# NjuHaoZhang/AMMCNet_AAAI2021

Hardware: AMD Instinct MI355X
Metric: frames/sec, 256x256x4 dual-stream clips (twostream forward, inference) (higher is better)
Workload: dtype f32-equivalent: (hi,lo) f16 split, 3 fp16 MFMAs per product (v_mfma_f32_32x32x16_f16 in the 4-wave k-half-major kernels, 16x16x32 in the 8-wave / fused-decoder kernels), f32 accumulate; 1 GPU; Ped2 full dual-stream + 2000-slot memory module, batch=16, inference (BASELINE.json configs[1]); batch_per_gpu=16, frame=256x256, n_embed=2000, embed_dim=64, k=2, parallelism=replicas x1 (no collective)

## Files before the change

ammcnet_aaai2021_amd/csrc/conv_outc_s16.hip:

```cpp
#include "ammc_common.h"
#include <hip/hip_fp16.h>
#include <stdio.h>
#include <stdlib.h>

namespace ammc_s16 {

typedef _Float16 f16x8o __attribute__((ext_vector_type(8)));

constexpr float O_LO_INV = 1.f / 2048.f;
constexpr int O_TH = 8, O_TW = 32, O_HW = O_TW + 2, O_HP = (O_TH + 2) * O_HW;
constexpr int O_APIECES = O_HP * 8;
constexpr int O_NT = 512;
constexpr int O_R = (O_APIECES + O_NT - 1) / O_NT;
constexpr int O_ASTAGE = ((O_APIECES + 63) / 64) * 64 * 4;
constexpr int O_MAXNS = 4;
constexpr int O_TG = O_MAXNS * 256;
constexpr int O_NS = 3;
constexpr int O_MAXCC = 2;
static_assert(O_R == 6, "OUTC_WAIT below knows 0, 2, 6 and 8 outstanding operations");

struct OutcArgs {
  AmmcConvDesc d;
  int tiles_x, tiles_y, ncc, kpad, total, nstore;
};

#define OUTC_WAIT(n)                                                              \
  switch (n) {                                                                    \
    case 0: asm volatile("s_waitcnt vmcnt(0)" ::: "memory"); break;               \
    case 2: asm volatile("s_waitcnt vmcnt(2)" ::: "memory"); break;               \
    case 6: asm volatile("s_waitcnt vmcnt(6)" ::: "memory"); break;               \
    default: asm volatile("s_waitcnt vmcnt(8)" ::: "memory"); break;              \
  }

__global__ __launch_bounds__(O_NT, 1) void conv_outc_s16_kernel(OutcArgs a) {
  extern __shared__ __attribute__((aligned(16))) float smem[];
  float* As = smem;
  float* Fs = smem + O_NS * O_ASTAGE;
  float* Tg = Fs + 9 * O_MAXCC * 128;
  float* Scr = Tg + 2 * O_TG;
  float* Sq = Scr + 256;

  const int tid = threadIdx.x, lane = tid & 63, wave = tid >> 6;
  const int l15 = lane & 15, g4 = lane >> 4;
  const AmmcConvDesc& d = a.d;
  const int G = gridDim.x;
  const int first = ammc_xcd_remap(blockIdx.x, G);
  const int ntile = (a.total - first + G - 1) / G;
  const int U = ntile * a.ncc;

  for (int i = tid; i < 9 * a.ncc * 32; i += O_NT) {
    const int chunk = i >> 5, row = (i >> 3) & 3, q = i & 7;
    int sl = q ^ row;
    sl ^= (sl >> 1) & 1;
    const f32x4 w = *reinterpret_cast<const f32x4*>(d.w + (int64_t)row * a.kpad + chunk * 32 + 4 * sl);
    *reinterpret_cast<f32x4*>(Fs + chunk * 128 + row * 32 + 4 * q) = w;
  }

  const int ns = a.nstore;
  const int64_t ycs = d.y_cs > 0 ? d.y_cs : 1;
  const bool score = d.sq_target != nullptr;

  float sc = 1.f, sh = 0.f;
  if (g4 < ns) {
    if (d.scale) sc = d.scale[g4];
    if (d.shift) sh = d.shift[g4];
  }
  asm volatile("" : "+v"(sc), "+v"(sh));

  int a_off[O_R];
#pragma unroll
  for (int j = 0; j < O_R; ++j) {
    int p = j * O_NT + tid;
    p = p < O_APIECES ? p : O_APIECES - 1;
    const int hp = p >> 3;
    int ls = (p & 7) ^ (hp & 7);
    ls ^= (ls >> 1) & 1;
    const int hy = hp / O_HW;
    const int hx = hp - hy * O_HW;
    a_off[j] = (int)((int64_t)hy * d.x_rs + (int64_t)hx * d.x_ps) + 4 * ls;
  }
#define OUTC_ISSUE(tile_, cc_, stage_)                                                                            \
  {                                                                                                               \
    int sp_ = (tile_);                                                                                            \
    const int tx_ = sp_ % a.tiles_x;                                                                              \
    sp_ /= a.tiles_x;                                                                                             \
    const int ty_ = sp_ % a.tiles_y;                                                                              \
    const int b_ = sp_ / a.tiles_y;                                                                               \
    const float* xp_ = d.x + ((int64_t)b_ * d.x_bs + (int64_t)(ty_ * O_TH) * d.x_rs + (int64_t)(tx_ * O_TW) * d.x_ps) + (cc_) * 32; \
    float* dst_ = As + (stage_) * O_ASTAGE + wave * 256;                                                          \
    _Pragma("unroll") for (int j = 0; j < O_R; ++j)                                                               \
      __builtin_amdgcn_global_load_lds(xp_ + a_off[j], (j * O_NT + wave * 64) * 4 < O_ASTAGE ? dst_ + j * O_NT * 4 : Scr, 16, 0, 0); \
  }
  const int tg_e0 = tid < ns * 256 ? tid : 0, tg_e1 = 512 + tid < ns * 256 ? 512 + tid : 0;
  const int64_t tg_o0 = (tg_e0 >> 8) * ycs + ((tg_e0 >> 5) & 7) * d.y_rs + (tg_e0 & 31) * d.y_ps;
  const int64_t tg_o1 = (tg_e1 >> 8) * ycs + ((tg_e1 >> 5) & 7) * d.y_rs + (tg_e1 & 31) * d.y_ps;
#define OUTC_ISSUE_TG(tile_, buf_)                                                                                \
  {                                                                                                               \
    int sp_ = (tile_);                                                                                            \
    const int tx_ = sp_ % a.tiles_x;                                                                              \
    sp_ /= a.tiles_x;                                                                                             \
    const int ty_ = sp_ % a.tiles_y;                                                                              \
    const int b_ = sp_ / a.tiles_y;                                                                               \
    const float* tp_ = d.sq_target + ((int64_t)b_ * d.y_bs + (int64_t)(ty_ * O_TH) * d.y_rs + (int64_t)(tx_ * O_TW) * d.y_ps); \
    __builtin_amdgcn_global_load_lds(tp_ + tg_o0, wave * 64 < ns * 256 ? Tg + (buf_) * O_TG + wave * 64 : Scr, 4, 0, 0);   \
    __builtin_amdgcn_global_load_lds(tp_ + tg_o1, 512 + wave * 64 < ns * 256 ? Tg + (buf_) * O_TG + 512 + wave * 64 : Scr, 4, 0, 0); \
  }

  int i_tile = first, i_cc = 0, i_stage = 0, issued = 0;
#define OUTC_ISSUE_NEXT()                                         \
  {                                                               \
    OUTC_ISSUE(i_tile, i_cc, i_stage);                            \
    ++issued;                                                     \
    i_stage = i_stage + 1 == O_NS ? 0 : i_stage + 1;              \
    if (++i_cc == a.ncc) i_cc = 0, i_tile += G;                   \
  }
  if (score && a.ncc == 1 && U > 0) OUTC_ISSUE_TG(first, 0);
  if (issued < U) OUTC_ISSUE_NEXT();
  if (issued < U) OUTC_ISSUE_NEXT();

  const int slot_hi = 2 * g4 + (g4 & 1), slot_lo = slot_hi ^ 1;
  const int frow = l15 & 3;
  const float* f_hi = Fs + frow * 32 + ((slot_hi ^ frow) << 2);
  const float* f_lo = Fs + frow * 32 + ((slot_lo ^ frow) << 2);
  const int hpb = wave * O_HW + l15;
  f32x4 acc[2], acx[2];
  acc[0] = acc[1] = acx[0] = acx[1] = f32x4{0.f, 0.f, 0.f, 0.f};
  int c_tile = first, c_cc = 0, c_stage = 0, c_par = 0;
  bool pend = false;
  int pend_b = 0;
  asm volatile("s_waitcnt lgkmcnt(0)" ::: "memory");

  for (int u = 0; u < U; ++u) {
    const int nwait = (u + 1 < U ? O_R : 0) + (pend ? 2 : 0);
    OUTC_WAIT(nwait);
    __builtin_amdgcn_s_barrier();
    asm volatile("" ::: "memory");
    if (pend && score && tid == 0) {
      float s = 0.f;
#pragma unroll
      for (int w = 0; w < 8; ++w) s += Sq[(c_par ^ 1) * 8 + w];
      unsafeAtomicAdd(d.sq_acc + pend_b, s);
    }
    const bool last_cc = c_cc + 1 == a.ncc;
    int sp = c_tile;
    const int tx = sp % a.tiles_x;
    sp /= a.tiles_x;
    const int ty = sp % a.tiles_y;
    const int b = sp / a.tiles_y;
    if (score && u + 1 < U && (a.ncc == 1 || c_cc + 2 == a.ncc)) {
      if (a.ncc == 1) OUTC_ISSUE_TG(c_tile + G, c_par ^ 1) else OUTC_ISSUE_TG(c_tile, c_par);
    }
    if (issued < U) OUTC_ISSUE_NEXT();

    const float* Ac = As + c_stage * O_ASTAGE;
    f16x8o fbh[2], fbl[2], fah[2][2], fal[2][2];
#define OUTC_LOAD(tap_, s_)                                                                   \
  {                                                                                           \
    const int chunk_ = (tap_) * a.ncc + c_cc;                                                 \
    fbh[s_] = *reinterpret_cast<const f16x8o*>(f_hi + chunk_ * 128);                          \
    fbl[s_] = *reinterpret_cast<const f16x8o*>(f_lo + chunk_ * 128);                          \
    _Pragma("unroll") for (int pt = 0; pt < 2; ++pt) {                                        \
      const int hp_ = hpb + 16 * pt + ((tap_) / 3) * O_HW + ((tap_) % 3);                     \
      const float* ap_ = Ac + hp_ * 32;                                                       \
      const int sw_ = hp_ & 7;                                                                \
      fah[s_][pt] = *reinterpret_cast<const f16x8o*>(ap_ + ((slot_hi ^ sw_) << 2));           \
      fal[s_][pt] = *reinterpret_cast<const f16x8o*>(ap_ + ((slot_lo ^ sw_) << 2));           \
    }                                                                                         \
  }
    OUTC_LOAD(0, 0);
#pragma unroll
    for (int tap = 0; tap < 9; ++tap) {
      const int cur = tap & 1;
      if (tap < 8) OUTC_LOAD(tap + 1, cur ^ 1);
      __builtin_amdgcn_sched_barrier(0);
#pragma unroll
      for (int pt = 0; pt < 2; ++pt) acc[pt] = __builtin_amdgcn_mfma_f32_16x16x32_f16(fbh[cur], fah[cur][pt], acc[pt], 0, 0, 0);
#pragma unroll
      for (int pt = 0; pt < 2; ++pt) acx[pt] = __builtin_amdgcn_mfma_f32_16x16x32_f16(fbl[cur], fah[cur][pt], acx[pt], 0, 0, 0);
#pragma unroll
      for (int pt = 0; pt < 2; ++pt) acx[pt] = __builtin_amdgcn_mfma_f32_16x16x32_f16(fbh[cur], fal[cur][pt], acx[pt], 0, 0, 0);
      __builtin_amdgcn_sched_barrier(0);
    }
#undef OUTC_LOAD

    pend = last_cc;
    if (last_cc) {
      const int y = ty * O_TH + wave, x0 = tx * O_TW;
      const int ch = g4 < ns ? g4 : 0;
      float sq0 = 0.f;
#pragma unroll
      for (int pt = 0; pt < 2; ++pt) {
        const f32x4 sum = acc[pt] + acx[pt] * O_LO_INV;
        const float r = g4 == 0 ? sum[0] : (g4 == 1 ? sum[1] : (g4 == 2 ? sum[2] : sum[3]));
        float t = r * sc + sh;
        if (d.act == AMMC_ACT_RELU) t = t > 0.f ? t : 0.f;
        else if (d.act == AMMC_ACT_TANH) t = tanhf(t);
        if (g4 < ns) {
          d.y[(int64_t)b * d.y_bs + (int64_t)y * d.y_rs + (int64_t)(x0 + 16 * pt + l15) * d.y_ps + (int64_t)ch * ycs] = t;
          if (score) {
            const float df = 0.5f * (Tg[c_par * O_TG + ch * 256 + wave * 32 + 16 * pt + l15] - t);
            sq0 += df * df;
          }
        }
        acc[pt] = acx[pt] = f32x4{0.f, 0.f, 0.f, 0.f};
      }
      if (score) {
#pragma unroll
        for (int off = 32; off > 0; off >>= 1) sq0 += __shfl_xor(sq0, off);
        if (lane == 0) Sq[c_par * 8 + wave] = sq0;
        asm volatile("s_waitcnt lgkmcnt(0)" ::: "memory");
      }
      pend_b = b;
    }
    c_stage = c_stage + 1 == O_NS ? 0 : c_stage + 1;
    if (++c_cc == a.ncc) c_cc = 0, c_tile += G, c_par ^= 1;
  }
  if (pend && score) {
    __builtin_amdgcn_s_barrier();
    asm volatile("" ::: "memory");
    if (tid == 0) {
      float s = 0.f;
#pragma unroll
      for (int w = 0; w < 8; ++w) s += Sq[(c_par ^ 1) * 8 + w];
      unsafeAtomicAdd(d.sq_acc + pend_b, s);
    }
  }
#undef OUTC_ISSUE
#undef OUTC_ISSUE_TG
#undef OUTC_ISSUE_NEXT
}

int conv_outc_s16_try(const AmmcConvDesc& d, int kpad, hipStream_t stream, char* label, int label_len) {
  constexpr int OUTC_SKIP = -12345;
  if (!(d.outc_stream ? d.outc_stream - 1 : ammc_opt_outc_stream())) return OUTC_SKIP;
  const int ns = d.n_store > 0 ? d.n_store : d.n;
  if (d.ntaps != 9 || d.up != 1 || d.x_step > 1 || !d.y_f32 || d.n != 32 || ns > O_MAXNS || d.res || d.pool_y) return OUTC_SKIP;
  if (d.cin % 32 || d.cin / 32 > O_MAXCC || d.width % O_TW || d.height % O_TH) return OUTC_SKIP;
  if (d.sq_target && !d.sq_acc) return AMMC_EINVAL;
  OutcArgs a;
  a.d = d;
  a.tiles_x = d.width / O_TW;
  a.tiles_y = d.height / O_TH;
  a.ncc = d.cin / 32;
  a.kpad = kpad;
  a.total = d.batch * a.tiles_y * a.tiles_x;
  a.nstore = ns;
  if (label) {
    snprintf(label, label_len, "conv_outc_s16");
    return AMMC_OK;
  }
  constexpr size_t lds = (size_t)(O_NS * O_ASTAGE + 9 * O_MAXCC * 128 + 2 * O_TG + 256 + 16) * sizeof(float);
  static_assert(lds <= 160 * 1024, "LDS budget");
  hipError_t e = hipFuncSetAttribute(reinterpret_cast<const void*>(conv_outc_s16_kernel),
                                     hipFuncAttributeMaxDynamicSharedMemorySize, (int)lds);
  if (e != hipSuccess) return (int)e;
  const int grid = a.total < 256 ? a.total : 256;
  hipLaunchKernelGGL(conv_outc_s16_kernel, dim3(grid), dim3(O_NT), lds, stream, a);
  return ammc_launch_status();
}

}
```

Measured before the change: 2443 frames/s.

## Restructure output conv as per-pixel tap-row GEMM with shuffle and LDS reduction

Result: no change. 2444 frames/s, median of 3 (+0.0%).

```diff
diff --git a/ammcnet_aaai2021_amd/csrc/conv_outc_s16.hip b/ammcnet_aaai2021_amd/csrc/conv_outc_s16.hip
--- a/ammcnet_aaai2021_amd/csrc/conv_outc_s16.hip
+++ b/ammcnet_aaai2021_amd/csrc/conv_outc_s16.hip
@@ -17,6 +17,12 @@
 constexpr int O_TG = O_MAXNS * 256;
 constexpr int O_NS = 3;
 constexpr int O_MAXCC = 2;
+constexpr int O_CPW = 3;
+constexpr int O_WP = 46;
+constexpr int O_XS = 272;
+constexpr int O_XFLOATS = 2 * 9 * O_XS;
+static_assert(O_WP + 2 <= O_CPW * 16 && 8 * O_WP >= O_HP, "every halo pixel is finished by a wave");
+static_assert(3 * O_MAXNS * O_XS <= O_XFLOATS, "exchange tile of four filters");
 static_assert(O_R == 6, "OUTC_WAIT below knows 0, 2, 6 and 8 outstanding operations");
 
 struct OutcArgs {
@@ -32,13 +38,16 @@
     default: asm volatile("s_waitcnt vmcnt(8)" ::: "memory"); break;              \
   }
 
+template <int NF, int NCC>
 __global__ __launch_bounds__(O_NT, 1) void conv_outc_s16_kernel(OutcArgs a) {
+  constexpr int NRT = (12 * NF + 15) / 16;
+  constexpr int NXB = NF <= 3 ? 2 : 1;
   extern __shared__ __attribute__((aligned(16))) float smem[];
   float* As = smem;
-  float* Fs = smem + O_NS * O_ASTAGE;
-  float* Tg = Fs + 9 * O_MAXCC * 128;
+  float* Tg = smem + O_NS * O_ASTAGE;
   float* Scr = Tg + 2 * O_TG;
   float* Sq = Scr + 256;
+  float* Xs = Sq + 16;
 
   const int tid = threadIdx.x, lane = tid & 63, wave = tid >> 6;
   const int l15 = lane & 15, g4 = lane >> 4;
@@ -46,15 +55,22 @@
   const int G = gridDim.x;
   const int first = ammc_xcd_remap(blockIdx.x, G);
   const int ntile = (a.total - first + G - 1) / G;
-  const int U = ntile * a.ncc;
-
-  for (int i = tid; i < 9 * a.ncc * 32; i += O_NT) {
-    const int chunk = i >> 5, row = (i >> 3) & 3, q = i & 7;
-    int sl = q ^ row;
-    sl ^= (sl >> 1) & 1;
-    const f32x4 w = *reinterpret_cast<const f32x4*>(d.w + (int64_t)row * a.kpad + chunk * 32 + 4 * sl);
-    *reinterpret_cast<f32x4*>(Fs + chunk * 128 + row * 32 + 4 * q) = w;
-  }
+  const int U = ntile * NCC;
+
+  f32x4 wh[NCC][NRT], wl[NCC][NRT];
+#pragma unroll
+  for (int cc = 0; cc < NCC; ++cc)
+#pragma unroll
+    for (int r = 0; r < NRT; ++r) {
+      const int row = 16 * r + l15, grp = row >> 2, dx = row & 3, dy = grp / NF, f = grp - dy * NF;
+      const bool real = dx < 3 && dy < 3;
+      const int tap = real ? 3 * dy + dx : 0;
+      const float* wp = d.w + (int64_t)f * a.kpad + (tap * NCC + cc) * 32 + 8 * g4;
+      f32x4 h = *reinterpret_cast<const f32x4*>(wp), l = *reinterpret_cast<const f32x4*>(wp + 4);
+      if (!real) h = l = f32x4{0.f, 0.f, 0.f, 0.f};
+      wh[cc][r] = h;
+      wl[cc][r] = l;
+    }
 
   const int ns = a.nstore;
   const int64_t ycs = d.y_cs > 0 ? d.y_cs : 1;
@@ -66,6 +82,10 @@
     if (d.shift) sh = d.shift[g4];
   }
   asm volatile("" : "+v"(sc), "+v"(sh));
+#pragma unroll
+  for (int cc = 0; cc < NCC; ++cc)
+#pragma unroll
+    for (int r = 0; r < NRT; ++r) asm volatile("" : "+v"(wh[cc][r]), "+v"(wl[cc][r]));
 
   int a_off[O_R];
 #pragma unroll
@@ -94,14 +114,9 @@
   const int tg_e0 = tid < ns * 256 ? tid : 0, tg_e1 = 512 + tid < ns * 256 ? 512 + tid : 0;
   const int64_t tg_o0 = (tg_e0 >> 8) * ycs + ((tg_e0 >> 5) & 7) * d.y_rs + (tg_e0 & 31) * d.y_ps;
   const int64_t tg_o1 = (tg_e1 >> 8) * ycs + ((tg_e1 >> 5) & 7) * d.y_rs + (tg_e1 & 31) * d.y_ps;
-#define OUTC_ISSUE_TG(tile_, buf_)                                                                                \
+#define OUTC_ISSUE_TG(b_, ty_, tx_, buf_)                                                                         \
   {                                                                                                               \
-    int sp_ = (tile_);                                                                                            \
-    const int tx_ = sp_ % a.tiles_x;                                                                              \
-    sp_ /= a.tiles_x;                                                                                             \
-    const int ty_ = sp_ % a.tiles_y;                                                                              \
-    const int b_ = sp_ / a.tiles_y;                                                                               \
-    const float* tp_ = d.sq_target + ((int64_t)b_ * d.y_bs + (int64_t)(ty_ * O_TH) * d.y_rs + (int64_t)(tx_ * O_TW) * d.y_ps); \
+    const float* tp_ = d.sq_target + ((int64_t)(b_) * d.y_bs + (int64_t)((ty_) * O_TH) * d.y_rs + (int64_t)((tx_) * O_TW) * d.y_ps); \
     __builtin_amdgcn_global_load_lds(tp_ + tg_o0, wave * 64 < ns * 256 ? Tg + (buf_) * O_TG + wave * 64 : Scr, 4, 0, 0);   \
     __builtin_amdgcn_global_load_lds(tp_ + tg_o1, 512 + wave * 64 < ns * 256 ? Tg + (buf_) * O_TG + 512 + wave * 64 : Scr, 4, 0, 0); \
   }
@@ -112,122 +127,167 @@
     OUTC_ISSUE(i_tile, i_cc, i_stage);                            \
     ++issued;                                                     \
     i_stage = i_stage + 1 == O_NS ? 0 : i_stage + 1;              \
-    if (++i_cc == a.ncc) i_cc = 0, i_tile += G;                   \
-  }
-  if (score && a.ncc == 1 && U > 0) OUTC_ISSUE_TG(first, 0);
+    if (++i_cc == NCC) i_cc = 0, i_tile += G;                     \
+  }
   if (issued < U) OUTC_ISSUE_NEXT();
   if (issued < U) OUTC_ISSUE_NEXT();
 
   const int slot_hi = 2 * g4 + (g4 & 1), slot_lo = slot_hi ^ 1;
-  const int frow = l15 & 3;
-  const float* f_hi = Fs + frow * 32 + ((slot_hi ^ frow) << 2);
-  const float* f_lo = Fs + frow * 32 + ((slot_lo ^ frow) << 2);
-  const int hpb = wave * O_HW + l15;
-  f32x4 acc[2], acx[2];
-  acc[0] = acc[1] = acx[0] = acx[1] = f32x4{0.f, 0.f, 0.f, 0.f};
-  int c_tile = first, c_cc = 0, c_stage = 0, c_par = 0;
-  bool pend = false;
-  int pend_b = 0;
-  asm volatile("s_waitcnt lgkmcnt(0)" ::: "memory");
-
-  for (int u = 0; u < U; ++u) {
-    const int nwait = (u + 1 < U ? O_R : 0) + (pend ? 2 : 0);
-    OUTC_WAIT(nwait);
-    __builtin_amdgcn_s_barrier();
-    asm volatile("" ::: "memory");
-    if (pend && score && tid == 0) {
-      float s = 0.f;
-#pragma unroll
-      for (int w = 0; w < 8; ++w) s += Sq[(c_par ^ 1) * 8 + w];
-      unsafeAtomicAdd(d.sq_acc + pend_b, s);
-    }
-    const bool last_cc = c_cc + 1 == a.ncc;
+  int a_hi[O_CPW], a_lo[O_CPW];
+  int xoff[O_CPW][NRT];
+#pragma unroll
+  for (int j = 0; j < O_CPW; ++j) {
+    const int col = 16 * j + l15, hp = O_WP * wave + col, hpc = hp < O_HP ? hp : O_HP - 1;
+    a_hi[j] = hpc * 32 + ((slot_hi ^ (hpc & 7)) << 2);
+    a_lo[j] = hpc * 32 + ((slot_lo ^ (hpc & 7)) << 2);
+    const int hy = hp / O_HW, hx = hp - hy * O_HW;
+#pragma unroll
+    for (int r = 0; r < NRT; ++r) {
+      const int grp = 4 * r + g4, dy = grp / NF, oy = hy - dy;
+      const bool ok = dy < 3 && col < O_WP && hp < O_HP && hx < O_TW && oy >= 0 && oy < O_TH;
+      xoff[j][r] = ok ? grp * O_XS + oy * O_TW + hx : -1;
+    }
+  }
+  const int src1 = (lane & 48) | ((l15 + 1) & 15), src2 = (lane & 48) | ((l15 + 2) & 15);
+
+  f32x4 acc[O_CPW][NRT], acx[O_CPW][NRT];
+#pragma unroll
+  for (int j = 0; j < O_CPW; ++j)
+#pragma unroll
+    for (int r = 0; r < NRT; ++r) acc[j][r] = acx[j][r] = f32x4{0.f, 0.f, 0.f, 0.f};
+
+#define OUTC_EPILOGUE(b_, ty_, tx_, par_)                                                                          \
+  {                                                                                                                \
+    const int y = (ty_) * O_TH + wave, x0 = (tx_) * O_TW;                                                          \
+    const int ch = g4 < ns ? g4 : 0;                                                                               \
+    const float* X = Xs + (NXB == 2 ? (par_) : 0) * (3 * NF * O_XS);                                               \
+    float sq0 = 0.f;                                                                                               \
+    _Pragma("unroll") for (int pt = 0; pt < 2; ++pt) {                                                             \
+      const float* xp = X + ch * O_XS + wave * O_TW + 16 * pt + l15;                                               \
+      const float r = (xp[0] + xp[NF * O_XS]) + xp[2 * NF * O_XS];                                                 \
+      float t = r * sc + sh;                                                                                       \
+      if (d.act == AMMC_ACT_RELU) t = t > 0.f ? t : 0.f;                                                           \
+      else if (d.act == AMMC_ACT_TANH) t = tanhf(t);                                                               \
+      if (g4 < ns) {                                                                                               \
+        d.y[(int64_t)(b_) * d.y_bs + (int64_t)y * d.y_rs + (int64_t)(x0 + 16 * pt + l15) * d.y_ps + (int64_t)ch * ycs] = t; \
+        if (score) {                                                                                               \
+          const float df = 0.5f * (Tg[(par_) * O_TG + ch * 256 + wave * 32 + 16 * pt + l15] - t);                  \
+          sq0 += df * df;                                                                                          \
+        }                                                                                                          \
+      }                                                                                                            \
+    }                                                                                                              \
+    if (score) {                                                                                                   \
+      _Pragma("unroll") for (int off = 32; off > 0; off >>= 1) sq0 += __shfl_xor(sq0, off);                        \
+      if (lane == 0) Sq[(par_) * 8 + wave] = sq0;                                                                  \
+    }                                                                                                              \
+    asm volatile("s_waitcnt lgkmcnt(0)" ::: "memory");                                                             \
+  }
+#define OUTC_ATOMIC(b_, par_)                                                                                      \
+  if (score && tid == 0) {                                \
+    float s = 0.f;                                                                                                 \
+    _Pragma("unroll") for (int w = 0; w < 8; ++w) s += Sq[(par_) * 8 + w];                                         \
+    unsafeAtomicAdd(d.sq_acc + (b_), s);                                                                           \
+  }
+
+  int c_tile = first, c_stage = 0, c_par = 0;
+  int u = 0;
+  bool stored = false;
+  bool sums = false;
+  int pb = 0, pty = 0, ptx = 0;
+  int sb = 0;
+
+  for (int k = 0; k < ntile; ++k) {
     int sp = c_tile;
     const int tx = sp % a.tiles_x;
     sp /= a.tiles_x;
     const int ty = sp % a.tiles_y;
     const int b = sp / a.tiles_y;
-    if (score && u + 1 < U && (a.ncc == 1 || c_cc + 2 == a.ncc)) {
-      if (a.ncc == 1) OUTC_ISSUE_TG(c_tile + G, c_par ^ 1) else OUTC_ISSUE_TG(c_tile, c_par);
-    }
-    if (issued < U) OUTC_ISSUE_NEXT();
-
-    const float* Ac = As + c_stage * O_ASTAGE;
-    f16x8o fbh[2], fbl[2], fah[2][2], fal[2][2];
-#define OUTC_LOAD(tap_, s_)                                                                   \
-  {                                                                                           \
-    const int chunk_ = (tap_) * a.ncc + c_cc;                                                 \
-    fbh[s_] = *reinterpret_cast<const f16x8o*>(f_hi + chunk_ * 128);                          \
-    fbl[s_] = *reinterpret_cast<const f16x8o*>(f_lo + chunk_ * 128);                          \
-    _Pragma("unroll") for (int pt = 0; pt < 2; ++pt) {                                        \
-      const int hp_ = hpb + 16 * pt + ((tap_) / 3) * O_HW + ((tap_) % 3);                     \
-      const float* ap_ = Ac + hp_ * 32;                                                       \
-      const int sw_ = hp_ & 7;                                                                \
-      fah[s_][pt] = *reinterpret_cast<const f16x8o*>(ap_ + ((slot_hi ^ sw_) << 2));           \
-      fal[s_][pt] = *reinterpret_cast<const f16x8o*>(ap_ + ((slot_lo ^ sw_) << 2));           \
-    }                                                                                         \
-  }
-    OUTC_LOAD(0, 0);
-#pragma unroll
-    for (int tap = 0; tap < 9; ++tap) {
-      const int cur = tap & 1;
-      if (tap < 8) OUTC_LOAD(tap + 1, cur ^ 1);
-      __builtin_amdgcn_sched_barrier(0);
-#pragma unroll
-      for (int pt = 0; pt < 2; ++pt) acc[pt] = __builtin_amdgcn_mfma_f32_16x16x32_f16(fbh[cur], fah[cur][pt], acc[pt], 0, 0, 0);
-#pragma unroll
-      for (int pt = 0; pt < 2; ++pt) acx[pt] = __builtin_amdgcn_mfma_f32_16x16x32_f16(fbl[cur], fah[cur][pt], acx[pt], 0, 0, 0);
-#pragma unroll
-      for (int pt = 0; pt < 2; ++pt) acx[pt] = __builtin_amdgcn_mfma_f32_16x16x32_f16(fbh[cur], fal[cur][pt], acx[pt], 0, 0, 0);
-      __builtin_amdgcn_sched_barrier(0);
-    }
-#undef OUTC_LOAD
-
-    pend = last_cc;
-    if (last_cc) {
-      const int y = ty * O_TH + wave, x0 = tx * O_TW;
-      const int ch = g4 < ns ? g4 : 0;
-      float sq0 = 0.f;
-#pragma unroll
-      for (int pt = 0; pt < 2; ++pt) {
-        const f32x4 sum = acc[pt] + acx[pt] * O_LO_INV;
-        const float r = g4 == 0 ? sum[0] : (g4 == 1 ? sum[1] : (g4 == 2 ? sum[2] : sum[3]));
-        float t = r * sc + sh;
-        if (d.act == AMMC_ACT_RELU) t = t > 0.f ? t : 0.f;
-        else if (d.act == AMMC_ACT_TANH) t = tanhf(t);
-        if (g4 < ns) {
-          d.y[(int64_t)b * d.y_bs + (int64_t)y * d.y_rs + (int64_t)(x0 + 16 * pt + l15) * d.y_ps + (int64_t)ch * ycs] = t;
-          if (score) {
-            const float df = 0.5f * (Tg[c_par * O_TG + ch * 256 + wave * 32 + 16 * pt + l15] - t);
-            sq0 += df * df;
+#pragma unroll
+    for (int cc = 0; cc < NCC; ++cc, ++u) {
+      const int nwait = (u + 1 < U ? O_R : 0) + (stored ? 2 : 0);
+      OUTC_WAIT(nwait);
+      __builtin_amdgcn_s_barrier();
+      asm volatile("" ::: "memory");
+      if (sums) OUTC_ATOMIC(sb, c_par ^ (cc == 0 ? 0 : 1));
+      sums = stored = false;
+      if (score && cc == 0) OUTC_ISSUE_TG(b, ty, tx, c_par);
+      if (issued < U) OUTC_ISSUE_NEXT();
+      if (cc == 0 && k > 0) {
+        OUTC_EPILOGUE(pb, pty, ptx, c_par ^ 1);
+        stored = true;
+        sums = score, sb = pb;
+      }
+
+      const float* Ac = As + c_stage * O_ASTAGE;
+      f16x8o fah[O_CPW], fal[O_CPW];
+#pragma unroll
+      for (int j = 0; j < O_CPW; ++j) {
+        fah[j] = *reinterpret_cast<const f16x8o*>(Ac + a_hi[j]);
+        fal[j] = *reinterpret_cast<const f16x8o*>(Ac + a_lo[j]);
+      }
+#pragma unroll
+      for (int j = 0; j < O_CPW; ++j) {
+#pragma unroll
+        for (int r = 0; r < NRT; ++r)
+          acc[j][r] = __builtin_amdgcn_mfma_f32_16x16x32_f16(__builtin_bit_cast(f16x8o, wh[cc][r]), fah[j], acc[j][r], 0, 0, 0);
+#pragma unroll
+        for (int r = 0; r < NRT; ++r)
+          acx[j][r] = __builtin_amdgcn_mfma_f32_16x16x32_f16(__builtin_bit_cast(f16x8o, wl[cc][r]), fah[j], acx[j][r], 0, 0, 0);
+#pragma unroll
+        for (int r = 0; r < NRT; ++r)
+          acx[j][r] = __builtin_amdgcn_mfma_f32_16x16x32_f16(__builtin_bit_cast(f16x8o, wh[cc][r]), fal[j], acx[j][r], 0, 0, 0);
+      }
+      c_stage = c_stage + 1 == O_NS ? 0 : c_stage + 1;
+    }
+
+    if (NXB == 1 && NCC == 1) {
+      __builtin_amdgcn_s_barrier();
+      asm volatile("" ::: "memory");
+    }
+    {
+      float* X = Xs + (NXB == 2 ? c_par : 0) * (3 * NF * O_XS);
+#pragma unroll
+      for (int r = 0; r < NRT; ++r) {
+        f32x4 sum[O_CPW];
+#pragma unroll
+        for (int j = 0; j < O_CPW; ++j) {
+          sum[j] = acc[j][r] + acx[j][r] * O_LO_INV;
+          acc[j][r] = acx[j][r] = f32x4{0.f, 0.f, 0.f, 0.f};
+        }
+#pragma unroll
+        for (int j = 0; j < O_CPW; ++j) {
+          float t1 = __shfl(sum[j][1], src1), t2 = __shfl(sum[j][2], src2);
+          if (j + 1 < O_CPW) {
+            const float n1 = __shfl(sum[j + 1][1], src1), n2 = __shfl(sum[j + 1][2], src2);
+            t1 = l15 < 15 ? t1 : n1;
+            t2 = l15 < 14 ? t2 : n2;
           }
+          const float s = (sum[j][0] + t1) + t2;
+          if (xoff[j][r] >= 0) X[xoff[j][r]] = s;
         }
-        acc[pt] = acx[pt] = f32x4{0.f, 0.f, 0.f, 0.f};
       }
-      if (score) {
-#pragma unroll
-        for (int off = 32; off > 0; off >>= 1) sq0 += __shfl_xor(sq0, off);
-        if (lane == 0) Sq[c_par * 8 + wave] = sq0;
-        asm volatile("s_waitcnt lgkmcnt(0)" ::: "memory");
-      }
-      pend_b = b;
-    }
-    c_stage = c_stage + 1 == O_NS ? 0 : c_stage + 1;
-    if (++c_cc == a.ncc) c_cc = 0, c_tile += G, c_par ^= 1;
-  }
-  if (pend && score) {
+    }
+    asm volatile("s_waitcnt lgkmcnt(0)" ::: "memory");
+    pb = b, pty = ty, ptx = tx;
+    c_tile += G, c_par ^= 1;
+  }
+  if (ntile > 0) {
+    asm volatile("s_waitcnt vmcnt(0)" ::: "memory");
     __builtin_amdgcn_s_barrier();
     asm volatile("" ::: "memory");
-    if (tid == 0) {
-      float s = 0.f;
-#pragma unroll
-      for (int w = 0; w < 8; ++w) s += Sq[(c_par ^ 1) * 8 + w];
-      unsafeAtomicAdd(d.sq_acc + pend_b, s);
+    if (sums) OUTC_ATOMIC(sb, c_par);
+    OUTC_EPILOGUE(pb, pty, ptx, c_par ^ 1);
+    if (score) {
+      __builtin_amdgcn_s_barrier();
+      asm volatile("" ::: "memory");
+      OUTC_ATOMIC(pb, c_par ^ 1);
     }
   }
 #undef OUTC_ISSUE
 #undef OUTC_ISSUE_TG
 #undef OUTC_ISSUE_NEXT
+#undef OUTC_EPILOGUE
+#undef OUTC_ATOMIC
 }
 
 int conv_outc_s16_try(const AmmcConvDesc& d, int kpad, hipStream_t stream, char* label, int label_len) {
@@ -249,13 +309,15 @@
     snprintf(label, label_len, "conv_outc_s16");
     return AMMC_OK;
   }
-  constexpr size_t lds = (size_t)(O_NS * O_ASTAGE + 9 * O_MAXCC * 128 + 2 * O_TG + 256 + 16) * sizeof(float);
+  constexpr size_t lds = (size_t)(O_NS * O_ASTAGE + 2 * O_TG + 256 + 16 + O_XFLOATS) * sizeof(float);
   static_assert(lds <= 160 * 1024, "LDS budget");
-  hipError_t e = hipFuncSetAttribute(reinterpret_cast<const void*>(conv_outc_s16_kernel),
-                                     hipFuncAttributeMaxDynamicSharedMemorySize, (int)lds);
+  void (*kern)(OutcArgs) = ns <= 2 ? (a.ncc == 1 ? conv_outc_s16_kernel<2, 1> : conv_outc_s16_kernel<2, 2>)
+                         : ns == 3 ? (a.ncc == 1 ? conv_outc_s16_kernel<3, 1> : conv_outc_s16_kernel<3, 2>)
+                                   : (a.ncc == 1 ? conv_outc_s16_kernel<4, 1> : conv_outc_s16_kernel<4, 2>);
+  hipError_t e = hipFuncSetAttribute(reinterpret_cast<const void*>(kern), hipFuncAttributeMaxDynamicSharedMemorySize, (int)lds);
   if (e != hipSuccess) return (int)e;
   const int grid = a.total < 256 ? a.total : 256;
-  hipLaunchKernelGGL(conv_outc_s16_kernel, dim3(grid), dim3(O_NT), lds, stream, a);
+  hipLaunchKernelGGL(kern, dim3(grid), dim3(O_NT), lds, stream, a);
   return ammc_launch_status();
 }
 
```
